# djamahl99/findnpropagate

Measured on AMD Instinct MI355X. Metric: NuScenes scenes/s (30k pts, Transfusion voxel backbone), higher is better.
Workload: dtype bf16

## Files before the change

findnpropagate_amd/csrc/rankgrid.h:

```cpp
#pragma once
#include "common.h"
#include <stdlib.h>

struct RankGridDims {
    int B, D, H, W;
    int bd, bh, bw;
    int th, tw;
};

__host__ __device__ inline RankGridDims fnp_make_dims(int B, int D, int H, int W) {
    RankGridDims g;
    g.B = B; g.D = D; g.H = H; g.W = W;
    g.bd = (D + 3) >> 2; g.bh = (H + 3) >> 2; g.bw = (W + 3) >> 2;
    g.th = (g.bh + 7) >> 3; g.tw = (g.bw + 7) >> 3;
    return g;
}

__host__ __device__ inline long long fnp_num_blocks(const RankGridDims &g) {
    return (long long)g.B * g.th * g.tw * 64 * g.bd;
}

struct RG {
    RankGridDims d;
    unsigned long long *bits;
// ... 141 lines not shown
    }
    __syncthreads();
    if (go.ctr) {
        if (tid < kCntTab && tab->cnt.key[tid] != 0u) {
            rg_count_global(go, tab->cnt.key[tid] - 1u, tab->cnt.val[tid]);
            tab->cnt.key[tid] = tab->cnt.val[tid] = 0u;
        }
        __syncthreads();
    }
}


__device__ __forceinline__ int rg_lookup(const RG &g, int b, int z, int y, int x) {
    const long long blk = rg_block_of(g.d, b, z, y, x);
    const unsigned long long w = g.bits[blk];
    const int bit = rg_bit_of(z, y, x);
    if (!((w >> bit) & 1ull)) return -1;
    const int r = (int)g.base[blk] + __popcll(w & ((1ull << bit) - 1ull));
    return g.perm ? g.perm[r] : r;
}

template <int KZ, int KY, int KX, bool DEFER = true>
__device__ __forceinline__ void nbr_row(const RG &g, int b, int loz, int loy, int lox, int *strip, int sstride, unsigned *mask_out = nullptr) {
    const int bz0 = loz >> 2, by0 = loy >> 2, bx0 = lox >> 2;
    unsigned long long w[2][2][2];
    unsigned base[2][2][2];
#pragma unroll
    for (int cy = 0; cy < 2; ++cy)
#pragma unroll
        for (int cx = 0; cx < 2; ++cx) {
            const int by = by0 + cy, bx = bx0 + cx;
            const bool need_yx = (cy == 0 || ((loy + KY - 1) >> 2) != by0) && (cx == 0 || ((lox + KX - 1) >> 2) != bx0);
            const bool in_yx = by >= 0 && by < g.d.bh && bx >= 0 && bx < g.d.bw;
            const unsigned col = (rg_morton3((unsigned)by & 7u) << 1) | rg_morton3((unsigned)bx & 7u);
            const long long colbase = ((((long long)b * g.d.th + (by >> 3)) * g.d.tw + (bx >> 3)) * 64 + col) * g.d.bd;
#pragma unroll
            for (int cz = 0; cz < 2; ++cz) {
                const int bz = bz0 + cz;
                const bool need = need_yx && (cz == 0 || ((loz + KZ - 1) >> 2) != bz0);
                const bool in = in_yx && bz >= 0 && bz < g.d.bd;
                unsigned long long ww = 0ull;
                unsigned bb = 0u;
                if (need && in) {
                    ww = g.bits[colbase + bz];
                    bb = g.base[colbase + bz];
                }
                w[cz][cy][cx] = ww;
                base[cz][cy][cx] = bb;
            }
        }
    constexpr int K = KZ * KY * KX;
    unsigned msk = 0u;
    int rk[DEFER ? K : 1];
    const int px0 = lox & 3;
    unsigned bitx[KX], mA[KX];
    bool selx[KX], vx[KX];
#pragma unroll
    for (int jx = 0; jx < KX; ++jx) {
        const int pj = px0 + jx, x = lox + jx;
        selx[jx] = pj >= 4;
        bitx[jx] = 1u << pj;
        mA[jx] = selx[jx] ? ((bitx[jx] - 1u) & 0xF0u) : (bitx[jx] - 1u);
        vx[jx] = x >= 0 && x < g.d.W;
    }
#pragma unroll
    for (int jz = 0; jz < KZ; ++jz) {
        const int z = loz + jz;
        const bool cz = (z >> 2) != bz0;
        const bool vz = z >= 0 && z < g.d.D;
        unsigned long long wz[2][2];
        unsigned bzv[2][2];
#pragma unroll
        for (int cy = 0; cy < 2; ++cy)
#pragma unroll
            for (int cx = 0; cx < 2; ++cx) {
                wz[cy][cx] = cz ? w[1][cy][cx] : w[0][cy][cx];
                bzv[cy][cx] = cz ? base[1][cy][cx] : base[0][cy][cx];
            }
#pragma unroll
        for (int jy = 0; jy < KY; ++jy) {
            const int y = loy + jy;
            const bool cy = (y >> 2) != by0;
            const bool vy = vz && y >= 0 && y < g.d.H;
            const unsigned long long wy0 = cy ? wz[1][0] : wz[0][0], wy1 = cy ? wz[1][1] : wz[0][1];
            const unsigned by0v = cy ? bzv[1][0] : bzv[0][0], by1v = cy ? bzv[1][1] : bzv[0][1];
            const int line = ((z & 3) << 4) | ((y & 3) << 2);
            const unsigned long long below = (1ull << line) - 1ull;
            const unsigned pre0 = by0v + (unsigned)__popcll(wy0 & below), pre1 = by1v + (unsigned)__popcll(wy1 & below);
            const unsigned lb = ((unsigned)(wy0 >> line) & 0xFu) | (((unsigned)(wy1 >> line) & 0xFu) << 4);
#pragma unroll
            for (int jx = 0; jx < KX; ++jx) {
                const bool hit = vy && vx[jx] && (lb & bitx[jx]) != 0u;
                const int r = (int)((selx[jx] ? pre1 : pre0) + (unsigned)__popc(lb & mA[jx]));
                const int e = (jz * KY + jy) * KX + jx;
                if constexpr (DEFER) {
                    rk[e] = hit ? r : -1;
                } else {
                    int rr = hit ? r : -1;
                    if (g.perm && hit) rr = g.perm[r];
                    strip[e * sstride] = rr;
                    if (mask_out && hit) msk |= 1u << (e & 31);
                }
            }
        }
    }
    if constexpr (DEFER) {
        if (g.perm) {
            int pr[K];
#pragma unroll
            for (int k = 0; k < K; ++k) pr[k] = g.perm[rk[k] < 0 ? 0 : rk[k]];
#pragma unroll
            for (int k = 0; k < K; ++k) rk[k] = rk[k] < 0 ? -1 : pr[k];
        }
#pragma unroll
        for (int k = 0; k < K; ++k) {
            strip[k * sstride] = rk[k];
            if (mask_out && rk[k] >= 0) msk |= 1u << (k & 31);
        }
    }
    if (mask_out) *mask_out = msk;
}


template <int K>
__device__ __forceinline__ void nbr_flush(const int *__restrict__ strip_wave, int o0, int n, int cap, int *__restrict__ nbr) {
    const int lane = fnp_lane();
    if ((cap & 3) == 0) {
#pragma unroll
        for (int j = 0; j < (K * 16 + 63) / 64; ++j) {
            const int e = j * 64 + lane, k = e >> 4, c = e & 15;
            if (k < K) {
                const int4 v = *reinterpret_cast<const int4 *>(strip_wave + k * 64 + c * 4);
                const int o = o0 + c * 4;
                if (o + 3 < n) *reinterpret_cast<int4 *>(nbr + (size_t)k * cap + o) = v;
                else {
                    if (o < n) nbr[(size_t)k * cap + o] = v.x;
                    if (o + 1 < n) nbr[(size_t)k * cap + o + 1] = v.y;
                    if (o + 2 < n) nbr[(size_t)k * cap + o + 2] = v.z;
                }
            }
        }
    } else {
#pragma unroll
        for (int k = 0; k < K; ++k)
            if (o0 + lane < n) nbr[(size_t)k * cap + o0 + lane] = strip_wave[k * 64 + lane];
    }
}


namespace fnp_scan {
constexpr int kTile = 4096;
int int32(const int *in, long long n, int *out, int *total, void *ws, hipStream_t s);
long long workspace_bytes(long long n);
int rank_grid(const RG &g, int *total, void *ws, hipStream_t s, int *out_coords = nullptr, int cap_out = 0, bool counted = false);
long long rank_grid_workspace_bytes(long long nsum);
}
```

findnpropagate_amd/csrc/scan.hip:

```cpp
#include "rankgrid.h"
#include <cstdint>
#include <type_traits>

namespace {

constexpr int kThreads = 256;
constexpr int kItems = fnp_scan::kTile / kThreads;

struct LoadInt {
    const int *p;
    __device__ __forceinline__ unsigned operator()(long long i) const { return (unsigned)p[i]; }
};

__device__ __forceinline__ unsigned wave_inclusive(unsigned v) {
    const int lane = fnp_lane();
#pragma unroll
    for (int d = 1; d < 64; d <<= 1) {
        const unsigned t = __shfl_up(v, d);
        if (lane >= d) v += t;
    }
    return v;
}

__device__ __forceinline__ unsigned block_exclusive(unsigned v, unsigned *wsum, unsigned &total) {
    const int wave = threadIdx.x >> 6, lane = fnp_lane();
    const unsigned inc = wave_inclusive(v);
    __syncthreads();
    if (lane == 63) wsum[wave] = inc;
    __syncthreads();
    unsigned off = 0;
#pragma unroll
    for (int w = 0; w < kThreads / 64; ++w) {
        const unsigned s = wsum[w];
        if (w < wave) off += s;
    }
    total = wsum[0] + wsum[1] + wsum[2] + wsum[3];
    return off + inc - v;
}

template <class L>
__global__ __launch_bounds__(kThreads) void tile_reduce_kernel(L load, long long n, unsigned *__restrict__ partial) {
    __shared__ unsigned wsum[4];
    const long long base = (long long)blockIdx.x * fnp_scan::kTile;
    unsigned s = 0;
#pragma unroll
    for (int j = 0; j < kItems; ++j) {
        const long long i = base + j * kThreads + threadIdx.x;
        if (i < n) s += load(i);
    }
    unsigned total;
    block_exclusive(s, wsum, total);
    if (threadIdx.x == 0) partial[blockIdx.x] = total;
}

__global__ __launch_bounds__(kThreads) void partial_scan_kernel(unsigned *__restrict__ partial, int np,
                                                                int *__restrict__ total_out) {
    __shared__ unsigned wsum[4];
    unsigned carry = 0;
    for (int base = 0; base < np; base += kThreads) {
        const int i = base + threadIdx.x;
        const unsigned v = i < np ? partial[i] : 0u;
        unsigned total;
        const unsigned ex = block_exclusive(v, wsum, total);
        if (i < np) partial[i] = carry + ex;
        carry += total;
    }
    if (threadIdx.x == 0) *total_out = (int)carry;
}

template <class L, class TOut>
__global__ __launch_bounds__(kThreads) void tile_scan_kernel(L load, long long n, const unsigned *__restrict__ partial,
                                                             TOut *__restrict__ out) {
    __shared__ unsigned wsum[4];
    const long long base = (long long)blockIdx.x * fnp_scan::kTile;
    unsigned carry = partial[blockIdx.x];
#pragma unroll 1
    for (int j = 0; j < kItems; ++j) {
        const long long i = base + j * kThreads + threadIdx.x;
        const unsigned v = i < n ? load(i) : 0u;
        unsigned total;
        const unsigned ex = block_exclusive(v, wsum, total);
        if (i < n) out[i] = (TOut)(carry + ex);
        carry += total;
    }
}

constexpr int kSmallTiles = 16;
__global__ __launch_bounds__(kThreads) void small_scan_kernel(const int *__restrict__ in, int n, int *__restrict__ out, int *__restrict__ total_out) {
    __shared__ unsigned wsum[4];
    const int base = blockIdx.x * fnp_scan::kTile;
    const int4 *in4 = reinterpret_cast<const int4 *>(in);
    unsigned s0 = 0, s1 = 0, s2 = 0, s3 = 0;
    for (int c = threadIdx.x; c < base / 4; c += 4 * kThreads) {
        const int4 a = in4[c];
        const int4 b = c + kThreads < base / 4 ? in4[c + kThreads] : make_int4(0, 0, 0, 0);
        const int4 d = c + 2 * kThreads < base / 4 ? in4[c + 2 * kThreads] : make_int4(0, 0, 0, 0);
        const int4 e = c + 3 * kThreads < base / 4 ? in4[c + 3 * kThreads] : make_int4(0, 0, 0, 0);
        s0 += (unsigned)(a.x + a.y + a.z + a.w);
        s1 += (unsigned)(b.x + b.y + b.z + b.w);
        s2 += (unsigned)(d.x + d.y + d.z + d.w);
        s3 += (unsigned)(e.x + e.y + e.z + e.w);
    }
    unsigned carry;
    block_exclusive(s0 + s1 + s2 + s3, wsum, carry);
    int4 v[kItems / 4];
#pragma unroll
    for (int j = 0; j < kItems / 4; ++j) {
        const int i = base + (j * kThreads + threadIdx.x) * 4;
        v[j] = make_int4(0, 0, 0, 0);
        if (i + 3 < n) v[j] = in4[i >> 2];
        else {
            if (i < n) v[j].x = in[i];
            if (i + 1 < n) v[j].y = in[i + 1];
            if (i + 2 < n) v[j].z = in[i + 2];
        }
    }
#pragma unroll
    for (int j = 0; j < kItems / 4; ++j) {
        const int i = base + (j * kThreads + threadIdx.x) * 4;
        unsigned tot;
        const unsigned ex = carry + block_exclusive((unsigned)(v[j].x + v[j].y + v[j].z + v[j].w), wsum, tot);
        const int4 o = make_int4((int)ex, (int)(ex + (unsigned)v[j].x), (int)(ex + (unsigned)(v[j].x + v[j].y)), (int)(ex + (unsigned)(v[j].x + v[j].y + v[j].z)));
        if (i + 3 < n) reinterpret_cast<int4 *>(out)[i >> 2] = o;
        else {
            if (i < n) out[i] = o.x;
            if (i + 1 < n) out[i + 1] = o.y;
            if (i + 2 < n) out[i + 2] = o.z;
        }
        carry += tot;
    }
    if (blockIdx.x == gridDim.x - 1 && threadIdx.x == 0) *total_out = (int)carry;
}

template <class L, class TOut>
int run_scan(L load, long long n, TOut *out, int *total, void *ws, hipStream_t s) {
    if (n < 0 || !total) return FNP_ERR_ARG;
    if (n == 0) {
        return fnp_fill_words(total, 1, 0u, s);
    }
    if (!out || !ws) return FNP_ERR_ARG;
    const int tiles = fnp_divup(n, fnp_scan::kTile);
    if constexpr (std::is_same<L, LoadInt>::value && std::is_same<TOut, int>::value) {
        if (tiles <= kSmallTiles && (const int *)out != load.p && (((uintptr_t)load.p | (uintptr_t)out) & 15) == 0) {
            hipLaunchKernelGGL(small_scan_kernel, dim3(tiles), dim3(kThreads), 0, s, load.p, (int)n, out, total);
            FNP_LAUNCH_CHECK();
            return FNP_OK;
        }
    }
    unsigned *partial = (unsigned *)ws;
    hipLaunchKernelGGL(HIP_KERNEL_NAME(tile_reduce_kernel<L>), dim3(tiles), dim3(kThreads), 0, s, load, n, partial);
    FNP_LAUNCH_CHECK();
    hipLaunchKernelGGL(partial_scan_kernel, dim3(1), dim3(kThreads), 0, s, partial, tiles, total);
    FNP_LAUNCH_CHECK();
    hipLaunchKernelGGL(HIP_KERNEL_NAME(tile_scan_kernel<L, TOut>), dim3(tiles), dim3(kThreads), 0, s, load, n, partial, out);
    FNP_LAUNCH_CHECK();
    return FNP_OK;
}

__device__ __forceinline__ unsigned wave_sum(unsigned v) {
#pragma unroll
    for (int d = 32; d >= 1; d >>= 1) v += __shfl_xor(v, d);
    return v;
}
__device__ __forceinline__ unsigned long long readlane64(unsigned long long v, int l) {
    const unsigned lo = __builtin_amdgcn_readlane((int)(unsigned)v, l), hi = __builtin_amdgcn_readlane((int)(unsigned)(v >> 32), l);
    return ((unsigned long long)hi << 32) | lo;
}

__global__ __launch_bounds__(kThreads) void rank_totals_kernel(const unsigned *__restrict__ cnt, long long nunits,
                                                               unsigned *__restrict__ gtot, unsigned *__restrict__ ctot) {
    __shared__ unsigned part[16];
    const int wave = threadIdx.x >> 6, lane = fnp_lane();
    const long long c = blockIdx.x;
#pragma unroll
    for (int i = 0; i < 4; ++i) {
        const long long grp = c * 16 + wave * 4 + i, U = grp * 64 + lane;
        const unsigned t = wave_sum(U < nunits ? cnt[U] : 0u);
        if (lane == 0) {
            part[wave * 4 + i] = t;
            if (grp * 64 < nunits) gtot[grp] = t;
        }
    }
    __syncthreads();
    if (threadIdx.x == 0) {
        unsigned t = 0;
#pragma unroll
        for (int i = 0; i < 16; ++i) t += part[i];
        ctot[c] = t;
    }
}

template <int PASS, int WPW>
__global__ __launch_bounds__(kThreads) void summary_pass_kernel(RG g, long long nunits, unsigned *__restrict__ cnt,
                                                                const unsigned *__restrict__ gtot,
                                                                const unsigned *__restrict__ ctot, int nchunks,
                                                                int *__restrict__ total, int cap_out,
                                                                int *__restrict__ out_coords) {
    constexpr int ROUND = WPW < 4 ? WPW : 4;
    const int lane = fnp_lane();
    const long long U = ((long long)fnp_xcd_block() * kThreads + threadIdx.x) >> 6;
    if (U >= nunits) return;
    if (PASS == 1 && U == 0) {
        unsigned t = 0;
        for (int c = lane; c < nchunks; c += 64) t += ctot[c];
        t = wave_sum(t);
        if (lane == 0) *total = (int)t;
    }
    const long long S0 = U * WPW;
    unsigned long long swl, todo;
    if (WPW == 1) {
        swl = g.summ[S0];
        todo = swl != 0ull ? 1ull : 0ull;
    } else {
        swl = (lane < WPW && S0 + lane < g.nsum) ? g.summ[S0 + lane] : 0ull;
        todo = __ballot(swl != 0ull);
    }
    if (todo == 0ull) {
        if (PASS == 0 && lane == 0) cnt[U] = 0u;
        return;
    }
    unsigned run = 0;
    if (PASS == 1) {
        const long long grp = U >> 6, chunk = U >> 10;
        unsigned p = 0;
        for (int i = lane; i < (int)chunk; i += 64) p += ctot[i];
        if (lane < (int)(grp - chunk * 16)) p += gtot[chunk * 16 + lane];
        if (lane < (int)(U - grp * 64)) p += cnt[grp * 64 + lane];
        run = wave_sum(p);
    }
    while (todo) {
        int j[ROUND];
        bool v[ROUND];
        unsigned long long bits[ROUND];
#pragma unroll
        for (int u = 0; u < ROUND; ++u) {
            v[u] = todo != 0ull;
            j[u] = v[u] ? __builtin_ctzll(todo) : 0;
            if (v[u]) todo &= todo - 1ull;
            const unsigned long long sw = WPW == 1 ? swl : readlane64(swl, j[u]);
            const bool occ = v[u] && ((sw >> lane) & 1ull);
            bits[u] = occ ? g.bits[(S0 + j[u]) * 64 + lane] : 0ull;
        }
#pragma unroll
        for (int u = 0; u < ROUND; ++u) {
            const unsigned c = (unsigned)__popcll(bits[u]);
            if (PASS == 0) {
                run += c;
            } else {
                if (!v[u]) break;
                const unsigned inc = wave_inclusive(c);
                const long long blk = (S0 + j[u]) * 64 + lane;
                int r = (int)(run + inc - c);
                if (bits[u]) {
                    g.base[blk] = (unsigned)r;
                    if (out_coords) {
                        int b, z0, y0, x0;
                        rg_decode(g.d, blk, 0, b, z0, y0, x0);
                        unsigned long long m = bits[u];
                        while (m) {
                            const int bit = __ffsll((long long)m) - 1;
                            m &= m - 1;
                            if (r < cap_out)
                                reinterpret_cast<int4 *>(out_coords)[r] = make_int4(b, z0 | (bit >> 4), y0 | ((bit >> 2) & 3), x0 | (bit & 3));
                            ++r;
                        }
                    }
                }
                if (WPW > 1) run += (unsigned)__builtin_amdgcn_readlane((int)inc, 63);
            }
        }
    }
    if (PASS == 0) {
        run = wave_sum(run);
        if (lane == 0) cnt[U] = run;
    }
}

}

namespace fnp_scan {
long long workspace_bytes(long long n) { return ((n + kTile - 1) / kTile + 1) * 4 + 64; }
int int32(const int *in, long long n, int *out, int *total, void *ws, hipStream_t s) {
    return run_scan(LoadInt{in}, n, out, total, ws, s);
}
long long rank_grid_workspace_bytes(long long nsum) {
    const long long ngroups = (nsum + 63) >> 6, nchunks = (nsum + 1023) >> 10;
    return ((nsum * 4 + 255) & ~255ll) + (((ngroups + nchunks) * 4 + 255) & ~255ll) + 256;
}
template <int WPW>
static int rank_grid_w(const RG &g, int *total, void *ws, hipStream_t s, int *out_coords, int cap_out, bool counted) {
    const long long nunits = (g.nsum + WPW - 1) / WPW;
    const long long ngroups = (nunits + 63) >> 6, nchunks = (nunits + 1023) >> 10;
    if (nchunks > 0x7fffffffll) return FNP_ERR_ARG;
    unsigned *cnt = (unsigned *)ws;
    unsigned *gtot = (unsigned *)((char *)ws + ((nunits * 4 + 255) & ~255ll));
    unsigned *ctot = gtot + ngroups;
    const int grid = fnp_divup(nunits * 64, kThreads);
    if (counted) {
        if (!g.ctr || g.wpw != WPW || g.nunits != nunits) return FNP_ERR_ARG;
        if (g.ctr_levels < 3) {
            hipLaunchKernelGGL(rank_totals_kernel, dim3((unsigned)nchunks), dim3(kThreads), 0, s, (const unsigned *)g.ctr, nunits, g.ctr + nunits,
                               g.ctr + nunits + ngroups);
            FNP_LAUNCH_CHECK();
        }
        hipLaunchKernelGGL(HIP_KERNEL_NAME(summary_pass_kernel<1, WPW>), dim3(grid), dim3(kThreads), 0, s, g, nunits, g.ctr,
                           (const unsigned *)(g.ctr + nunits), (const unsigned *)(g.ctr + nunits + ngroups), (int)nchunks, total, cap_out, out_coords);
        FNP_LAUNCH_CHECK();
        return FNP_OK;
    }
    hipLaunchKernelGGL(HIP_KERNEL_NAME(summary_pass_kernel<0, WPW>), dim3(grid), dim3(kThreads), 0, s, g, nunits, cnt,
                       (const unsigned *)nullptr, (const unsigned *)nullptr, (int)nchunks, total, 0, (int *)nullptr);
    FNP_LAUNCH_CHECK();
    hipLaunchKernelGGL(rank_totals_kernel, dim3((unsigned)nchunks), dim3(kThreads), 0, s, (const unsigned *)cnt, nunits, gtot, ctot);
    FNP_LAUNCH_CHECK();
    hipLaunchKernelGGL(HIP_KERNEL_NAME(summary_pass_kernel<1, WPW>), dim3(grid), dim3(kThreads), 0, s, g, nunits, cnt,
                       (const unsigned *)gtot, (const unsigned *)ctot, (int)nchunks, total, cap_out, out_coords);
    FNP_LAUNCH_CHECK();
    return FNP_OK;
}
int rank_grid(const RG &g, int *total, void *ws, hipStream_t s, int *out_coords, int cap_out, bool counted) {
    const int wpw = g.wpw;
    if (wpw == 64) return rank_grid_w<64>(g, total, ws, s, out_coords, cap_out, counted);
    if (wpw == 16) return rank_grid_w<16>(g, total, ws, s, out_coords, cap_out, counted);
    if (wpw == 8) return rank_grid_w<8>(g, total, ws, s, out_coords, cap_out, counted);
    return rank_grid_w<1>(g, total, ws, s, out_coords, cap_out, counted);
}
}

extern "C" int64_t fnp_rankgrid_counter_words(int B, int D, int H, int W) {
    if (B <= 0 || D <= 0 || H <= 0 || W <= 0) return 0;
    const long long nblk = fnp_num_blocks(fnp_make_dims(B, D, H, W));
    return fnp_rg_counter_words((nblk + 63) >> 6) + 64;
}

extern "C" int64_t fnp_rankgrid_workspace_bytes(int B, int D, int H, int W) {
    if (B <= 0 || D <= 0 || H <= 0 || W <= 0) return 0;
    const long long nblk = fnp_num_blocks(fnp_make_dims(B, D, H, W));
    return fnp_scan::rank_grid_workspace_bytes((nblk + 63) >> 6) + 256;
}
```

findnpropagate_amd/csrc/voxelize.hip:

```cpp
#include "rankgrid.h"

namespace {

constexpr int kThreads = 256;
constexpr int kSentinel = 0x7f7f7f7f;
constexpr int kMaxBatch = 1024;

struct VoxWs {
    long long *code;
    int *rank;
    int *flag;
    int *top;
    int *cnt;
    int *scene;
    int *n_sorted;
    int *n_first;
    int *fscan;
    void *scan_ws;
};

__host__ long long align_up(long long v) { return (v + 255) & ~255ll; }

__host__ long long carve(VoxWs &w, char *base, long long n, int B, int cap, int maxp, long long nsum) {
    long long off = 0;
    auto take = [&](long long bytes) {
        char *p = base ? base + off : nullptr;
        off += align_up(bytes);
        return p;
    };
    w.code = (long long *)take(8 * n);
    w.rank = (int *)take(4 * n);
    w.flag = (int *)take(4 * n);
    w.fscan = (int *)take(4 * n);
    w.top = (int *)take(4ll * cap * maxp);
    w.cnt = (int *)take(4ll * cap + 4);
    w.scene = (int *)take(4ll * (3 * B + 8));
    w.n_sorted = (int *)take(4);
    w.n_first = (int *)take(4);
    const long long a = fnp_scan::rank_grid_workspace_bytes(nsum), b2 = fnp_scan::workspace_bytes(n);
    w.scan_ws = take(a > b2 ? a : b2);
    return off;
}

__device__ __forceinline__ int batch_of(const int *__restrict__ off, int B, int i) {
    int lo = 0, hi = B;
    while (hi - lo > 1) {
        const int mid = (lo + hi) >> 1;
        if (off[mid] <= i) lo = mid; else hi = mid;
    }
    return lo;
}

__global__ __launch_bounds__(kThreads) void vox_mark_kernel(const float *__restrict__ pts, int n, int C,
                                                            const int *__restrict__ boff, int B, fnp_voxel_cfg cfg,
                                                            RG g, long long *__restrict__ code, int *__restrict__ cnt) {
    {
        const int z = blockIdx.x * kThreads + threadIdx.x;
        if (z <= n) cnt[z] = 0;
        if (z == 0 && (long long)gridDim.x * kThreads <= n) cnt[n] = 0;
    }
    __shared__ MarkTab tab;
    mark_tab_init(&tab, threadIdx.x, kThreads);
    const int i = blockIdx.x * kThreads + threadIdx.x;
    const int lane = fnp_lane();
    long long blk = -1;
    unsigned long long m = 0ull;
    if (i < n) {
        const float *p = pts + (size_t)i * C;
        int c[3];
        bool ok = true;
#pragma unroll
        for (int j = 0; j < 3; ++j) {
            const float q = (p[j] - cfg.range_min[j]) / cfg.voxel_size[j];
            const float f = floorf(q);
            ok = ok && (f >= 0.f) && (f < (float)cfg.grid[j]);
            c[j] = (int)f;
        }
        long long cd = -1;
        if (ok) {
            const int i0 = __builtin_amdgcn_readfirstlane(i);
            int b = batch_of(boff, B, i0);
            if (b + 1 < B && i >= boff[b + 1]) b = batch_of(boff, B, i);
            blk = rg_block_of(g.d, b, c[2], c[1], c[0]);
            const int bit = rg_bit_of(c[2], c[1], c[0]);
            m = 1ull << bit;
            cd = (blk << 6) | bit;
        }
        code[i] = cd;
    }
#pragma unroll
    for (int d = 1; d < 64; d <<= 1) {
        const long long nb = __shfl_up(blk, d);
        const unsigned long long nm = __shfl_up(m, d);
        if (lane >= d && nb == blk) m |= nm;
    }
    const long long nxt = __shfl_down(blk, 1);
    if (blk >= 0 && (lane == 63 || nxt != blk)) mark_put(&tab, g, blk, m);
    mark_tab_flush(&tab, g, threadIdx.x, kThreads);
}

__global__ __launch_bounds__(kThreads) void vox_insert_kernel(int n, int maxp, int cap,
                                                              const unsigned long long *__restrict__ bits,
                                                              const unsigned *__restrict__ base,
                                                              const long long *__restrict__ code,
                                                              int *__restrict__ rank, int *__restrict__ top, int *__restrict__ cnt,
                                                              int *__restrict__ crowded, int *__restrict__ late) {
    const int i = blockIdx.x * kThreads + threadIdx.x;
    if (i >= n) return;
    late[i] = 0;
    const long long cd = code[i];
    int r = -1;
    if (cd >= 0) {
        const long long blk = cd >> 6;
        const int bit = (int)(cd & 63);
        r = (int)base[blk] + __popcll(bits[blk] & ((1ull << bit) - 1ull));
        if (r >= cap) r = -1;
    }
    rank[i] = r;
    if (r < 0) return;
    const int s = atomicAdd(&cnt[r], 1);
    if (s < maxp) {
        top[(size_t)r * maxp + s] = i;
    } else {
        late[i] = 1;
        if (s == maxp) *crowded = 1;
    }
}

__global__ __launch_bounds__(kThreads) void vox_crowded_insert_kernel(int n, int maxp, const int *__restrict__ rank, const int *__restrict__ late,
                                                                     int *__restrict__ top, const int *__restrict__ crowded) {
    if (*crowded == 0) return;
    const int i = blockIdx.x * kThreads + threadIdx.x;
    if (i >= n || late[i] == 0) return;
    int carry = i;
    int *slots = top + (size_t)rank[i] * maxp;
    for (int j = 0; j < maxp; ++j) {
        const int old = atomicMin(&slots[j], carry);
        carry = old > carry ? old : carry;
    }
}

__global__ __launch_bounds__(kThreads) void vox_flag_kernel(int n, int maxp, const int *__restrict__ rank,
                                                            const int *__restrict__ top, const int *__restrict__ cnt, int *__restrict__ flag) {
    const int i = fnp_xcd_block() * kThreads + threadIdx.x;
    if (i >= n) return;
    const int r = rank[i];
    int f = 0;
    if (r >= 0) {
        const int np = min(cnt[r], maxp);
        int m = kSentinel;
        for (int j = 0; j < np; ++j) m = min(m, top[(size_t)r * maxp + j]);
        f = m == i ? 1 : 0;
    }
    flag[i] = f;
}

__global__ __launch_bounds__(64) void vox_scene_kernel(const int *__restrict__ boff, int B, int n, const int *__restrict__ fc,
                                                       const int *__restrict__ n_first, int max_voxels, int cap,
                                                       int *__restrict__ scene, int *__restrict__ n_voxels) {
    int *fc_start = scene;
    int *out_base = scene + (B + 1);
    const int lane = threadIdx.x;
    const int total = *n_first;
    int acc = 0;
    for (int b0 = 0; b0 < B; b0 += 64) {
        const int b = b0 + lane;
        int c = 0;
        if (b < B) {
            const int o0 = boff[b], o1 = boff[b + 1];
            const int f0 = (o0 < n) ? fc[o0] : total, f1 = (o1 < n) ? fc[o1] : total;
            fc_start[b] = f0;
            if (b == B - 1) fc_start[B] = f1;
            c = min(f1 - f0, max_voxels);
        }
        int inc = c;
#pragma unroll
        for (int d = 1; d < 64; d <<= 1) {
            const int t = __shfl_up(inc, d);
            if (lane >= d) inc += t;
        }
        if (b < B) out_base[b] = acc + inc - c;
        acc += __shfl(inc, 63);
    }
    if (lane == 0) {
        out_base[B] = acc;
        scene[2 * (B + 1)] = 0;
        *n_voxels = acc;
    }
}

struct CellPts {
    const int *slots;
    int np, s0, s1;
    __device__ __forceinline__ int next_above(int prev) const {
        if (np <= 2) {
            const int a = s0, b = np == 2 ? s1 : kSentinel;
            const int lo = a < b ? a : b, hi = a < b ? b : a;
            return lo > prev ? lo : hi;
        }
        int m = kSentinel;
        for (int j = 0; j < np; ++j) {
            const int v = slots[j];
            m = (v > prev && v < m) ? v : m;
        }
        return m;
    }
};

__device__ __forceinline__ void vox_write_row(const float *__restrict__ pts, int C, int maxp, const CellPts &cp, int p0, int r, int id,
                                              int bb, int z, int y, int x, int *__restrict__ perm, int *__restrict__ coords,
                                              int *__restrict__ num_points, float *__restrict__ mean, float *__restrict__ voxels) {
    const int np = cp.np;
    auto next_above = [&](int prev) -> int { return cp.next_above(prev); };
    perm[r] = id;
    reinterpret_cast<int4 *>(coords)[id] = make_int4(bb, z, y, x);
    num_points[id] = np;
    const float norm = (float)(np < 1 ? 1 : np);
    if ((C == 5 || C == 4) && maxp < 16) {
        typedef float f4u __attribute__((ext_vector_type(4), aligned(4)));
        f4u s4 = {0.f, 0.f, 0.f, 0.f};
        float part[4] = {0.f, 0.f, 0.f, 0.f}, tl[3] = {0.f, 0.f, 0.f};
        const int P4 = maxp & ~3;
        int pi = p0;
        for (int j = 0; j < np; ++j) {
            const float *pr = pts + (size_t)pi * C;
            const f4u v4 = *reinterpret_cast<const f4u *>(pr);
            const float v1 = C == 5 ? pr[4] : 0.f;
            if (j + 1 < np) pi = next_above(pi);
            s4 += v4;
#pragma unroll
            for (int k = 0; k < 4; ++k) part[k] += (j < P4 && (j & 3) == k) ? v1 : 0.f;
#pragma unroll
            for (int k = 0; k < 3; ++k) tl[k] = (j == P4 + k) ? v1 : tl[k];
        }
        float *mo = mean + (size_t)id * C;
        f4u m4 = {s4[0] / norm, s4[1] / norm, s4[2] / norm, s4[3] / norm};
        *reinterpret_cast<f4u *>(mo) = m4;
        if (C == 5) {
            float s1f = part[0];
#pragma unroll
            for (int k = 0; k < 3; ++k) s1f += (P4 + k < maxp) ? tl[k] : 0.f;
            s1f += part[1];
            s1f += part[2];
            s1f += part[3];
            mo[4] = s1f / norm;
        }
    } else {
        for (int c = 0; c < C; ++c) {
            const bool ilp = C < 8 && c >= (C / 4) * 4;
            const int nsum = ilp ? 4 : 1, size = ilp ? maxp / 4 : maxp;
            int lp = 0;
            while ((1 << lp) < size) ++lp;
            lp = C >= 8 ? 30 : max(4, lp / 4);
            const int mask = (1 << lp) - 1;
            float acc[4][4];
#pragma unroll
            for (int k = 0; k < 4; ++k)
#pragma unroll
                for (int l = 0; l < 4; ++l) acc[k][l] = 0.f;
            float tail = 0.f;
            bool tail_started = false;
            int pi = p0;
            for (int j = 0; j < maxp; ++j) {
                const float v = j < np ? pts[(size_t)pi * C + c] : 0.f;
                if (j + 1 < np) pi = next_above(pi);
                if (j < size * nsum) {
                    const int e = j / nsum + 1;
#pragma unroll
                    for (int k = 0; k < 4; ++k) {
                        if (k != (ilp ? (j & 3) : 0)) continue;
                        acc[k][0] += v;
                        if ((e & mask) == 0) {
#pragma unroll
                            for (int l = 1; l < 4; ++l) {
                                acc[k][l] += acc[k][l - 1];
                                acc[k][l - 1] = 0.f;
                                if ((e & (mask << (l * lp))) != 0) break;
                            }
                        }
                    }
                } else {
                    if (!tail_started) {
#pragma unroll
                        for (int l = 1; l < 4; ++l) acc[0][0] += acc[0][l];
                        tail = acc[0][0];
                        tail_started = true;
                    }
                    tail += v;
                }
            }
            float sacc;
            if (ilp) {
                if (!tail_started) {
#pragma unroll
                    for (int l = 1; l < 4; ++l) acc[0][0] += acc[0][l];
                    tail = acc[0][0];
                }
                sacc = tail;
#pragma unroll
                for (int k = 1; k < 4; ++k) {
#pragma unroll
                    for (int l = 1; l < 4; ++l) acc[k][0] += acc[k][l];
                    sacc += acc[k][0];
                }
            } else {
#pragma unroll
                for (int l = 1; l < 4; ++l) acc[0][0] += acc[0][l];
// ... 24 lines not shown
                                                                   float *__restrict__ voxels, int *__restrict__ n_cells,
                                                                   int *__restrict__ n_dropped) {
    const int ns = min(*n_sorted, cap);
    const int *fc_start = scene;
    const int *out_base = scene + (B + 1);
    if (n_cells && blockIdx.x == 0 && threadIdx.x == 0) *n_cells = ns;
    for (int r = ns + blockIdx.x * kThreads + threadIdx.x; r < cap; r += gridDim.x * kThreads) perm[r] = -1;
    const int i = (int)fnp_xcd_block() * kThreads + threadIdx.x;
    if (i >= n) return;
    const int r = rank[i];
    if (r < 0) return;
    const int f0 = fc[i], f1 = i + 1 < n ? fc[i + 1] : *n_first;
    if (f1 == f0) return;
    const long long cd = code[i];
    int bb, z, y, x;
    rg_decode(g, cd >> 6, (int)(cd & 63), bb, z, y, x);
    const int srank = f0 - fc_start[bb];
    const int id = out_base[bb] + srank;
    if (srank >= max_voxels || id >= cap) {
        perm[r] = -1;
        if (n_cells) {
            const int t = out_base[B] + atomicAdd(n_dropped, 1);
            if (t < cap) reinterpret_cast<int4 *>(coords)[t] = make_int4(bb, z, y, x);
        }
        return;
    }
    CellPts cp;
    cp.slots = top + (size_t)r * maxp;
    cp.np = min(cnt[r], maxp);
    cp.s0 = i;
    cp.s1 = kSentinel;
    if (cp.np == 2) {
        const int a = cp.slots[0], b = cp.slots[1];
        cp.s1 = a == i ? b : a;
    }
    vox_write_row(pts, C, maxp, cp, i, r, id, bb, z, y, x, perm, coords, num_points, mean, voxels);
}

__device__ __forceinline__ bool coord_ok(const RankGridDims &g, const int4 &c) {
    return c.x >= 0 && c.x < g.B && c.y >= 0 && c.y < g.D && c.z >= 0 && c.z < g.H && c.w >= 0 && c.w < g.W;
}

__device__ __forceinline__ void rg_zero_counters(const RG &g, long long first, long long stride) {
    if (!g.ctr) return;
    const long long words = g.nunits + ((g.nunits + 63) >> 6) + ((g.nunits + 1023) >> 10);
    for (long long i = first; i < words; i += stride) g.ctr[i] = 0u;
}

template <bool CLEAR>
__global__ __launch_bounds__(kThreads) void rg_mark_coords_kernel(const int *__restrict__ coords,
                                                                  const int *__restrict__ n_rows, int cap, RG g) {
    const int n = min(*n_rows, cap);
    for (int i = blockIdx.x * kThreads + threadIdx.x; i < n; i += gridDim.x * kThreads) {
        const int4 c = reinterpret_cast<const int4 *>(coords)[i];
        if (!coord_ok(g.d, c)) continue;
        const long long blk = rg_block_of(g.d, c.x, c.y, c.z, c.w);
        if (CLEAR) {
            g.bits[blk] = 0ull;
            g.summ[blk >> 6] = 0ull;
        } else {
            rg_mark(g, blk, rg_bit_of(c.y, c.z, c.w));
        }
    }
    if (CLEAR) rg_zero_counters(g, (long long)blockIdx.x * kThreads + threadIdx.x, (long long)gridDim.x * kThreads);
}

__global__ __launch_bounds__(kThreads) void rg_perm_kernel(const int *__restrict__ coords, const int *__restrict__ n_rows,
                                                           int cap, RG g) {
    const int n = min(*n_rows, cap);
    RG lookup = g;
    lookup.perm = nullptr;
    for (int i = blockIdx.x * kThreads + threadIdx.x; i < n; i += gridDim.x * kThreads) {
        const int4 c = reinterpret_cast<const int4 *>(coords)[i];
        if (!coord_ok(g.d, c)) continue;
        const int r = rg_lookup(lookup, c.x, c.y, c.z, c.w);
        if (r >= 0 && r < cap) g.perm[r] = i;
    }
}

}

extern "C" int64_t fnp_rankgrid_num_blocks(int B, int D, int H, int W) {
    if (B <= 0 || D <= 0 || H <= 0 || W <= 0) return 0;
    return fnp_num_blocks(fnp_make_dims(B, D, H, W));
}
extern "C" int64_t fnp_rankgrid_num_summary(int B, int D, int H, int W) {
    return (fnp_rankgrid_num_blocks(B, D, H, W) + 63) >> 6;
}

static bool grid_covers(const fnp_voxel_cfg *cfg, const fnp_rankgrid *g) {
    return g->D >= cfg->grid[2] && g->H >= cfg->grid[1] && g->W >= cfg->grid[0];
}

extern "C" int64_t fnp_voxelize_workspace_bytes(int64_t n_points, const fnp_voxel_cfg *cfg, const fnp_rankgrid *grid) {
    if (!cfg || n_points < 0 || !grid || grid->B <= 0 || !grid_covers(cfg, grid)) return FNP_ERR_ARG;
    VoxWs w;
    const RankGridDims g = fnp_make_dims(grid->B, grid->D, grid->H, grid->W);
    const long long n = n_points > 0 ? n_points : 1;
    return carve(w, nullptr, n, grid->B, (int)n, cfg->max_points, (fnp_num_blocks(g) + 63) >> 6);
}

__global__ __launch_bounds__(kThreads) void stage_points_kernel(const float *__restrict__ src, long long n_words, long long n_prev_words, float pad,
                                                                float *__restrict__ dst, const int *__restrict__ off_src, int n_off,
                                                                int *__restrict__ off_dst) {
    const long long i = (long long)blockIdx.x * kThreads + threadIdx.x;
    if (i < n_words) dst[i] = src[i];
    else if (i < n_prev_words) dst[i] = pad;
    if (i < n_off) off_dst[i] = off_src[i];
}
extern "C" int fnp_stage_points(const float *points, int64_t n_points, int64_t n_prev_points, int num_features, float pad, float *dst_points,
                                const int *batch_offsets, int n_offsets, int *dst_offsets, fnp_stream_t stream) {
    if (n_points < 0 || n_prev_points < 0 || num_features <= 0 || !dst_points || n_offsets < 0 || (n_points > 0 && !points) ||
        (n_offsets > 0 && (!batch_offsets || !dst_offsets)))
        return FNP_ERR_ARG;
    const long long nw = (long long)n_points * num_features, pw = (long long)n_prev_points * num_features;
    const long long span = nw > pw ? nw : pw;
    const long long items = span > n_offsets ? span : n_offsets;
    if (items == 0) return FNP_OK;
    if (items > (long long)kThreads * 0x7fffffff) return FNP_ERR_ARG;
    hipLaunchKernelGGL(stage_points_kernel, dim3((unsigned)((items + kThreads - 1) / kThreads)), dim3(kThreads), 0, (hipStream_t)stream, points, nw, pw, pad,
                       dst_points, batch_offsets, n_offsets, dst_offsets);
    FNP_LAUNCH_CHECK();
    return FNP_OK;
}

extern "C" int fnp_voxelize(const float *points, int n, const int *batch_offsets, const fnp_voxel_cfg *cfg,
                            const fnp_rankgrid *grid, void *workspace, int64_t workspace_bytes, int *coords,
                            int *num_points, float *mean_feats, float *voxels, int *n_voxels, int *n_cells, int cap,
                            fnp_stream_t stream) {
    hipStream_t s = (hipStream_t)stream;
    if (!cfg || n < 0 || cap <= 0 || !n_voxels || !fnp_rg_valid(grid, true) || grid->B > kMaxBatch || !grid_covers(cfg, grid))
        return FNP_ERR_ARG;
    if (cfg->num_features < 3 || cfg->max_points <= 0 || cfg->max_points > 64 || cfg->max_voxels <= 0) return FNP_ERR_ARG;
    if (n == 0) {
        int frc = fnp_fill_words(n_voxels, 1, 0u, s);
        if (!frc && n_cells) frc = fnp_fill_words(n_cells, 1, 0u, s);
        return frc;
    }
    if (!points || !batch_offsets || !workspace || !coords || !num_points || !mean_feats) return FNP_ERR_ARG;
    if (cap < n) return FNP_ERR_ARG;
    const RG g = fnp_rg_view(grid);
    const int B = grid->B;
    VoxWs w;
    const long long need = carve(w, (char *)workspace, n, B, n, cfg->max_points, g.nsum);
    if (need > workspace_bytes) return FNP_ERR_WORKSPACE;
    const int maxp = cfg->max_points, C = cfg->num_features;
    const int pgrid = fnp_divup(n, kThreads);

    hipLaunchKernelGGL(vox_mark_kernel, dim3(pgrid), dim3(kThreads), 0, s, points, n, C, batch_offsets, B, *cfg, g, w.code, w.cnt);
    FNP_LAUNCH_CHECK();
    int rc = fnp_scan::rank_grid(g, w.n_sorted, w.scan_ws, s, nullptr, 0, g.ctr != nullptr);
    if (rc) return rc;
    hipLaunchKernelGGL(vox_insert_kernel, dim3(pgrid), dim3(kThreads), 0, s, n, maxp, n,
                       (const unsigned long long *)g.bits, (const unsigned *)g.base, w.code, w.rank, w.top, w.cnt, w.cnt + n, w.flag);
    FNP_LAUNCH_CHECK();
    hipLaunchKernelGGL(vox_crowded_insert_kernel, dim3(pgrid), dim3(kThreads), 0, s, n, maxp, (const int *)w.rank, (const int *)w.flag, w.top, (const int *)(w.cnt + n));
    FNP_LAUNCH_CHECK();
    hipLaunchKernelGGL(vox_flag_kernel, dim3(pgrid), dim3(kThreads), 0, s, n, maxp, w.rank, w.top, (const int *)w.cnt, w.flag);
    FNP_LAUNCH_CHECK();
    rc = fnp_scan::int32(w.flag, n, w.fscan, w.n_first, w.scan_ws, s);
    if (rc) return rc;
    hipLaunchKernelGGL(vox_scene_kernel, dim3(1), dim3(64), 0, s, batch_offsets, B, n, w.fscan, w.n_first,
                       cfg->max_voxels, cap, w.scene, n_voxels);
    FNP_LAUNCH_CHECK();
    hipLaunchKernelGGL(vox_emit_points_kernel, dim3(pgrid), dim3(kThreads), 0, s, points, n, C, maxp, batch_offsets, B, cfg->max_voxels,
                       g.d, w.code, (const int *)w.rank, w.top, (const int *)w.cnt, w.fscan, (const int *)w.n_first, w.scene, w.n_sorted, n,
                       g.perm, coords, num_points, mean_feats, voxels, n_cells, w.scene + 2 * (B + 1));
    FNP_LAUNCH_CHECK();
    return FNP_OK;
}

extern "C" int fnp_rankgrid_build(const int *coords, const int *n_rows, int cap, const fnp_rankgrid *grid,
                                  void *workspace, int64_t workspace_bytes, fnp_stream_t stream) {
    hipStream_t s = (hipStream_t)stream;
    if (!coords || !n_rows || cap <= 0 || !fnp_rg_valid(grid) || !workspace) return FNP_ERR_ARG;
    const RG g = fnp_rg_view(grid);
    if (fnp_scan::rank_grid_workspace_bytes(g.nsum) + 256 > workspace_bytes) return FNP_ERR_WORKSPACE;
    int *total = (int *)workspace;
    void *scan_ws = (char *)workspace + 256;
    const int blocks = fnp_grid_for(cap, kThreads);
    hipLaunchKernelGGL(rg_mark_coords_kernel<false>, dim3(blocks), dim3(kThreads), 0, s, coords, n_rows, cap, g);
    FNP_LAUNCH_CHECK();
    int rc = fnp_scan::rank_grid(g, total, scan_ws, s);
    if (rc) return rc;
    if (g.perm) {
        {
            const int frc = fnp_fill_words(g.perm, cap, 0xffffffffu, s);
            if (frc) return frc;
        }
        hipLaunchKernelGGL(rg_perm_kernel, dim3(blocks), dim3(kThreads), 0, s, coords, n_rows, cap, g);
        FNP_LAUNCH_CHECK();
    }
    return FNP_OK;
}

extern "C" int fnp_rankgrid_clear(const int *coords, const int *n_rows, int cap, const fnp_rankgrid *grid,
                                  fnp_stream_t stream) {
    if (!coords || !n_rows || cap <= 0 || !fnp_rg_valid(grid)) return FNP_ERR_ARG;
    const RG g = fnp_rg_view(grid);
    hipLaunchKernelGGL(rg_mark_coords_kernel<true>, dim3(fnp_grid_for(cap, kThreads)), dim3(kThreads), 0,
                       (hipStream_t)stream, coords, n_rows, cap, g);
    FNP_LAUNCH_CHECK();
    return FNP_OK;
}

struct ClearJob {
    const int *coords, *n_rows;
    int cap;
    RG g;
};
struct ClearJobs { ClearJob j[8]; };

__global__ __launch_bounds__(kThreads) void rg_clear_multi_kernel(ClearJobs jobs) {
    const ClearJob &J = jobs.j[blockIdx.y];
    const int n = min(*J.n_rows, J.cap);
    for (int i = fnp_xcd_block() * kThreads + threadIdx.x; i < n; i += gridDim.x * kThreads) {
        const int4 c = reinterpret_cast<const int4 *>(J.coords)[i];
        if (!coord_ok(J.g.d, c)) continue;
        const long long blk = rg_block_of(J.g.d, c.x, c.y, c.z, c.w);
        J.g.bits[blk] = 0ull;
        J.g.summ[blk >> 6] = 0ull;
    }
    rg_zero_counters(J.g, blockIdx.x * kThreads + threadIdx.x, gridDim.x * kThreads);
}

extern "C" int fnp_rankgrid_clear_multi(int count, const int *const *coords, const int *const *n_rows, const int *caps,
                                        const fnp_rankgrid *grids, fnp_stream_t stream) {
    if (count <= 0 || count > 8 || !coords || !n_rows || !caps || !grids) return FNP_ERR_ARG;
    ClearJobs jobs{};
    int cap_max = 1;
    for (int i = 0; i < count; ++i) {
        if (!coords[i] || !n_rows[i] || caps[i] <= 0 || !fnp_rg_valid(&grids[i])) return FNP_ERR_ARG;
        jobs.j[i].coords = coords[i];
        jobs.j[i].n_rows = n_rows[i];
        jobs.j[i].cap = caps[i];
        jobs.j[i].g = fnp_rg_view(&grids[i]);
        if (caps[i] > cap_max) cap_max = caps[i];
    }
    const int gx = (fnp_grid_for(cap_max, kThreads, 512) + 7) & ~7;
    hipLaunchKernelGGL(rg_clear_multi_kernel, dim3(gx, count), dim3(kThreads), 0, (hipStream_t)stream, jobs);
    FNP_LAUNCH_CHECK();
    return FNP_OK;
}

__device__ __forceinline__ unsigned long long clr_readlane64(unsigned long long v, int l) {
    const unsigned lo = __builtin_amdgcn_readlane((int)(unsigned)v, l), hi = __builtin_amdgcn_readlane((int)(unsigned)(v >> 32), l);
    return ((unsigned long long)hi << 32) | lo;
}
__global__ __launch_bounds__(kThreads) void rg_clear_summary_kernel(ClearJobs jobs) {
    const RG &g = jobs.j[blockIdx.y].g;
    const int lane = fnp_lane();
    const long long nunits = (g.nsum + 63) >> 6, wstride = (long long)gridDim.x * (kThreads / 64);
    for (long long U = (long long)blockIdx.x * (kThreads / 64) + (threadIdx.x >> 6); U < nunits; U += wstride) {
        const long long S0 = U * 64;
        const unsigned long long sw = (S0 + lane < g.nsum) ? g.summ[S0 + lane] : 0ull;
        unsigned long long todo = __ballot(sw != 0ull);
        if (todo == 0ull) continue;
        while (todo) {
            const int j = __builtin_ctzll(todo);
            todo &= todo - 1ull;
            const unsigned long long swj = clr_readlane64(sw, j);
            if ((swj >> lane) & 1ull) g.bits[(S0 + j) * 64 + lane] = 0ull;
        }
        if (sw != 0ull) g.summ[S0 + lane] = 0ull;
    }
    rg_zero_counters(g, (long long)blockIdx.x * kThreads + threadIdx.x, (long long)gridDim.x * kThreads);
}

extern "C" int fnp_rankgrid_clear_summary(int count, const fnp_rankgrid *grids, fnp_stream_t stream) {
    if (count <= 0 || count > 8 || !grids) return FNP_ERR_ARG;
    ClearJobs jobs{};
    long long units_max = 1;
    for (int i = 0; i < count; ++i) {
        if (!fnp_rg_valid(&grids[i])) return FNP_ERR_ARG;
        jobs.j[i].g = fnp_rg_view(&grids[i]);
        const long long u = (jobs.j[i].g.nsum + 63) >> 6;
        if (u > units_max) units_max = u;
    }
    const int gx = (fnp_grid_for(units_max, kThreads / 64, 2048) + 7) & ~7;
    hipLaunchKernelGGL(rg_clear_summary_kernel, dim3(gx, count), dim3(kThreads), 0, (hipStream_t)stream, jobs);
    FNP_LAUNCH_CHECK();
    return FNP_OK;
}

#include <vector>

extern "C" int fnp_host_voxelize(const float *points, int n, const fnp_voxel_cfg *cfg, float *voxels, int *coords,
                                 int *num_points, int max_rows) {
    if (!cfg || n < 0 || max_rows < 0 || cfg->num_features < 3 || cfg->max_points <= 0 || (n > 0 && !points)) return FNP_ERR_ARG;
    if (n > 0 && max_rows > 0 && (!voxels || !coords || !num_points)) return FNP_ERR_ARG;
    const int C = cfg->num_features, P = cfg->max_points;
    const int cap_rows = cfg->max_voxels < max_rows ? cfg->max_voxels : max_rows;
    size_t tbl = 64;
    while (tbl < (size_t)(n > 0 ? n : 1) * 2) tbl <<= 1;
    std::vector<long long> keys(tbl, -1ll);
    std::vector<int> vals(tbl, 0);
    int m = 0;
    for (int i = 0; i < n; ++i) {
        const float *p = points + (size_t)i * C;
        int c[3];
        bool ok = true;
        for (int j = 0; j < 3; ++j) {
            const float q = (p[j] - cfg->range_min[j]) / cfg->voxel_size[j];
            const float f = floorf(q);
            ok = ok && (f >= 0.f) && (f < (float)cfg->grid[j]);
            c[j] = (int)f;
        }
        if (!ok) continue;
        const long long key = ((long long)c[2] * cfg->grid[1] + c[1]) * cfg->grid[0] + c[0];
        size_t h = (size_t)((unsigned long long)key * 0x9E3779B97F4A7C15ull) & (tbl - 1);
        while (keys[h] != -1ll && keys[h] != key) h = (h + 1) & (tbl - 1);
        int row;
        if (keys[h] == key) {
// ... 21 lines not shown
```

Measured before the change: 14030.

## Compact late points, fuse flag with tile sums, and self-compute small rank totals

Insert now appends overflowing points to a compact list with one wave-aggregated atomic per wave. The crowded-insert pass walks only that list with a capped grid and skips points that cannot displace a slot. When the flag scan needs more than one launch, the flag kernel also writes per-tile sums so the scan's reduce pass can be skipped. For small grids the rank pass computes prefix totals from the raw counts, dropping the separate totals kernel. These changes cut launches and full-array passes, at the cost of an extra workspace buffer and O(U) prefix loops per wave in the self-total path.

```diff
diff --git a/findnpropagate_amd/csrc/rankgrid.h b/findnpropagate_amd/csrc/rankgrid.h
--- a/findnpropagate_amd/csrc/rankgrid.h
+++ b/findnpropagate_amd/csrc/rankgrid.h
@@ -317,6 +317,9 @@
 constexpr int kTile = 4096;
 int int32(const int *in, long long n, int *out, int *total, void *ws, hipStream_t s);
 long long workspace_bytes(long long n);
+bool int32_is_one_launch(const int *in, long long n, const int *out);
+unsigned *tile_sums(void *ws);
+int int32_from_tile_sums(const int *in, long long n, int *out, int *total, void *ws, hipStream_t s);
 int rank_grid(const RG &g, int *total, void *ws, hipStream_t s, int *out_coords = nullptr, int cap_out = 0, bool counted = false);
 long long rank_grid_workspace_bytes(long long nsum);
 }
diff --git a/findnpropagate_amd/csrc/scan.hip b/findnpropagate_amd/csrc/scan.hip
--- a/findnpropagate_amd/csrc/scan.hip
+++ b/findnpropagate_amd/csrc/scan.hip
@@ -132,8 +132,12 @@
     if (blockIdx.x == gridDim.x - 1 && threadIdx.x == 0) *total_out = (int)carry;
 }
 
+bool small_scan_fits(const int *in, long long n, const int *out) {
+    return n > 0 && fnp_divup(n, fnp_scan::kTile) <= kSmallTiles && out != in && (((uintptr_t)in | (uintptr_t)out) & 15) == 0;
+}
+
 template <class L, class TOut>
-int run_scan(L load, long long n, TOut *out, int *total, void *ws, hipStream_t s) {
+int run_scan(L load, long long n, TOut *out, int *total, void *ws, hipStream_t s, bool have_sums = false) {
     if (n < 0 || !total) return FNP_ERR_ARG;
     if (n == 0) {
         return fnp_fill_words(total, 1, 0u, s);
@@ -141,15 +145,17 @@
     if (!out || !ws) return FNP_ERR_ARG;
     const int tiles = fnp_divup(n, fnp_scan::kTile);
     if constexpr (std::is_same<L, LoadInt>::value && std::is_same<TOut, int>::value) {
-        if (tiles <= kSmallTiles && (const int *)out != load.p && (((uintptr_t)load.p | (uintptr_t)out) & 15) == 0) {
+        if (!have_sums && small_scan_fits(load.p, n, (const int *)out)) {
             hipLaunchKernelGGL(small_scan_kernel, dim3(tiles), dim3(kThreads), 0, s, load.p, (int)n, out, total);
             FNP_LAUNCH_CHECK();
             return FNP_OK;
         }
     }
     unsigned *partial = (unsigned *)ws;
-    hipLaunchKernelGGL(HIP_KERNEL_NAME(tile_reduce_kernel<L>), dim3(tiles), dim3(kThreads), 0, s, load, n, partial);
-    FNP_LAUNCH_CHECK();
+    if (!have_sums) {
+        hipLaunchKernelGGL(HIP_KERNEL_NAME(tile_reduce_kernel<L>), dim3(tiles), dim3(kThreads), 0, s, load, n, partial);
+        FNP_LAUNCH_CHECK();
+    }
     hipLaunchKernelGGL(partial_scan_kernel, dim3(1), dim3(kThreads), 0, s, partial, tiles, total);
     FNP_LAUNCH_CHECK();
     hipLaunchKernelGGL(HIP_KERNEL_NAME(tile_scan_kernel<L, TOut>), dim3(tiles), dim3(kThreads), 0, s, load, n, partial, out);
@@ -200,9 +206,11 @@
     const int lane = fnp_lane();
     const long long U = ((long long)fnp_xcd_block() * kThreads + threadIdx.x) >> 6;
     if (U >= nunits) return;
+    const bool self_totals = PASS == 1 && gtot == nullptr;
     if (PASS == 1 && U == 0) {
         unsigned t = 0;
-        for (int c = lane; c < nchunks; c += 64) t += ctot[c];
+        if (self_totals) for (long long u = lane; u < nunits; u += 64) t += cnt[u];
+        else for (int c = lane; c < nchunks; c += 64) t += ctot[c];
         t = wave_sum(t);
         if (lane == 0) *total = (int)t;
     }
@@ -223,9 +231,13 @@
     if (PASS == 1) {
         const long long grp = U >> 6, chunk = U >> 10;
         unsigned p = 0;
-        for (int i = lane; i < (int)chunk; i += 64) p += ctot[i];
-        if (lane < (int)(grp - chunk * 16)) p += gtot[chunk * 16 + lane];
-        if (lane < (int)(U - grp * 64)) p += cnt[grp * 64 + lane];
+        if (self_totals) {
+            for (long long u = lane; u < U; u += 64) p += cnt[u];
+        } else {
+            for (int i = lane; i < (int)chunk; i += 64) p += ctot[i];
+            if (lane < (int)(grp - chunk * 16)) p += gtot[chunk * 16 + lane];
+            if (lane < (int)(U - grp * 64)) p += cnt[grp * 64 + lane];
+        }
         run = wave_sum(p);
     }
     while (todo) {
@@ -283,10 +295,16 @@
 int int32(const int *in, long long n, int *out, int *total, void *ws, hipStream_t s) {
     return run_scan(LoadInt{in}, n, out, total, ws, s);
 }
+bool int32_is_one_launch(const int *in, long long n, const int *out) { return small_scan_fits(in, n, out); }
+unsigned *tile_sums(void *ws) { return (unsigned *)ws; }
+int int32_from_tile_sums(const int *in, long long n, int *out, int *total, void *ws, hipStream_t s) {
+    return run_scan(LoadInt{in}, n, out, total, ws, s, true);
+}
 long long rank_grid_workspace_bytes(long long nsum) {
     const long long ngroups = (nsum + 63) >> 6, nchunks = (nsum + 1023) >> 10;
     return ((nsum * 4 + 255) & ~255ll) + (((ngroups + nchunks) * 4 + 255) & ~255ll) + 256;
 }
+constexpr long long kSelfTotalUnits = 1024;
 template <int WPW>
 static int rank_grid_w(const RG &g, int *total, void *ws, hipStream_t s, int *out_coords, int cap_out, bool counted) {
     const long long nunits = (g.nsum + WPW - 1) / WPW;
@@ -298,13 +316,15 @@
     const int grid = fnp_divup(nunits * 64, kThreads);
     if (counted) {
         if (!g.ctr || g.wpw != WPW || g.nunits != nunits) return FNP_ERR_ARG;
-        if (g.ctr_levels < 3) {
+        const bool self_totals = g.ctr_levels < 3 && nunits <= kSelfTotalUnits;
+        if (g.ctr_levels < 3 && !self_totals) {
             hipLaunchKernelGGL(rank_totals_kernel, dim3((unsigned)nchunks), dim3(kThreads), 0, s, (const unsigned *)g.ctr, nunits, g.ctr + nunits,
                                g.ctr + nunits + ngroups);
             FNP_LAUNCH_CHECK();
         }
         hipLaunchKernelGGL(HIP_KERNEL_NAME(summary_pass_kernel<1, WPW>), dim3(grid), dim3(kThreads), 0, s, g, nunits, g.ctr,
-                           (const unsigned *)(g.ctr + nunits), (const unsigned *)(g.ctr + nunits + ngroups), (int)nchunks, total, cap_out, out_coords);
+                           self_totals ? (const unsigned *)nullptr : (const unsigned *)(g.ctr + nunits), (const unsigned *)(g.ctr + nunits + ngroups),
+                           (int)nchunks, total, cap_out, out_coords);
         FNP_LAUNCH_CHECK();
         return FNP_OK;
     }
diff --git a/findnpropagate_amd/csrc/voxelize.hip b/findnpropagate_amd/csrc/voxelize.hip
--- a/findnpropagate_amd/csrc/voxelize.hip
+++ b/findnpropagate_amd/csrc/voxelize.hip
@@ -12,6 +12,7 @@
     int *flag;
     int *top;
     int *cnt;
+    int *late;
     int *scene;
     int *n_sorted;
     int *n_first;
@@ -34,6 +35,7 @@
     w.fscan = (int *)take(4 * n);
     w.top = (int *)take(4ll * cap * maxp);
     w.cnt = (int *)take(4ll * cap + 4);
+    w.late = (int *)take(4 * n);
     w.scene = (int *)take(4ll * (3 * B + 8));
     w.n_sorted = (int *)take(4);
     w.n_first = (int *)take(4);
@@ -104,55 +106,94 @@
                                                               const unsigned *__restrict__ base,
                                                               const long long *__restrict__ code,
                                                               int *__restrict__ rank, int *__restrict__ top, int *__restrict__ cnt,
-                                                              int *__restrict__ crowded, int *__restrict__ late) {
+                                                              int *__restrict__ n_late, int *__restrict__ late) {
     const int i = blockIdx.x * kThreads + threadIdx.x;
-    if (i >= n) return;
-    late[i] = 0;
-    const long long cd = code[i];
-    int r = -1;
-    if (cd >= 0) {
-        const long long blk = cd >> 6;
-        const int bit = (int)(cd & 63);
-        r = (int)base[blk] + __popcll(bits[blk] & ((1ull << bit) - 1ull));
-        if (r >= cap) r = -1;
-    }
-    rank[i] = r;
-    if (r < 0) return;
-    const int s = atomicAdd(&cnt[r], 1);
-    if (s < maxp) {
-        top[(size_t)r * maxp + s] = i;
-    } else {
-        late[i] = 1;
-        if (s == maxp) *crowded = 1;
-    }
-}
-
+    bool is_late = false;
+    if (i < n) {
+        const long long cd = code[i];
+        int r = -1;
+        if (cd >= 0) {
+            const long long blk = cd >> 6;
+            const int bit = (int)(cd & 63);
+            r = (int)base[blk] + __popcll(bits[blk] & ((1ull << bit) - 1ull));
+            if (r >= cap) r = -1;
+        }
+        rank[i] = r;
+        if (r >= 0) {
+            const int s = atomicAdd(&cnt[r], 1);
+            if (s < maxp) top[(size_t)r * maxp + s] = i;
+            else is_late = true;
+        }
+    }
+    const unsigned long long lm = __ballot(is_late);
+    if (lm == 0ull) return;
+    const int lane = fnp_lane(), leader = __builtin_ctzll(lm);
+    int at = 0;
+    if (lane == leader) at = atomicAdd(n_late, __popcll(lm));
+    at = __shfl(at, leader);
+    if (is_late) late[at + __popcll(lm & ((1ull << lane) - 1ull))] = i;
+}
+
+constexpr int kLateBlocks = 128;
 __global__ __launch_bounds__(kThreads) void vox_crowded_insert_kernel(int n, int maxp, const int *__restrict__ rank, const int *__restrict__ late,
-                                                                     int *__restrict__ top, const int *__restrict__ crowded) {
-    if (*crowded == 0) return;
-    const int i = blockIdx.x * kThreads + threadIdx.x;
-    if (i >= n || late[i] == 0) return;
-    int carry = i;
-    int *slots = top + (size_t)rank[i] * maxp;
-    for (int j = 0; j < maxp; ++j) {
-        const int old = atomicMin(&slots[j], carry);
-        carry = old > carry ? old : carry;
-    }
-}
-
+                                                                     int *__restrict__ top, const int *__restrict__ n_late) {
+    const int nl = min(*n_late, n);
+    for (int k = blockIdx.x * kThreads + threadIdx.x; k < nl; k += gridDim.x * kThreads) {
+        const int i = late[k];
+        int carry = i;
+        int *slots = top + (size_t)rank[i] * maxp;
+        int mx = -1;
+        for (int j = 0; j < maxp; ++j) mx = max(mx, slots[j]);
+        if (i > mx) continue;
+        for (int j = 0; j < maxp; ++j) {
+            const int old = atomicMin(&slots[j], carry);
+            carry = old > carry ? old : carry;
+        }
+    }
+}
+
+__device__ __forceinline__ int vox_is_first(int i, int r, int np, int maxp, const int *__restrict__ top) {
+    int m = kSentinel;
+    for (int j = 0; j < np; ++j) m = min(m, top[(size_t)r * maxp + j]);
+    return m == i ? 1 : 0;
+}
 __global__ __launch_bounds__(kThreads) void vox_flag_kernel(int n, int maxp, const int *__restrict__ rank,
                                                             const int *__restrict__ top, const int *__restrict__ cnt, int *__restrict__ flag) {
     const int i = fnp_xcd_block() * kThreads + threadIdx.x;
     if (i >= n) return;
     const int r = rank[i];
-    int f = 0;
-    if (r >= 0) {
-        const int np = min(cnt[r], maxp);
-        int m = kSentinel;
-        for (int j = 0; j < np; ++j) m = min(m, top[(size_t)r * maxp + j]);
-        f = m == i ? 1 : 0;
-    }
-    flag[i] = f;
+    flag[i] = r >= 0 ? vox_is_first(i, r, min(cnt[r], maxp), maxp, top) : 0;
+}
+constexpr int kFlagThreads = 1024, kFlagItems = fnp_scan::kTile / kFlagThreads;
+__global__ __launch_bounds__(kFlagThreads) void vox_flag_tiles_kernel(int n, int maxp, const int *__restrict__ rank,
+                                                                      const int *__restrict__ top, const int *__restrict__ cnt, int *__restrict__ flag,
+                                                                      unsigned *__restrict__ tile_sum) {
+    __shared__ unsigned wsum[kFlagThreads / 64];
+    const unsigned tile = fnp_xcd_block();
+    const long long base = (long long)tile * fnp_scan::kTile + threadIdx.x;
+    int r[kFlagItems], np[kFlagItems];
+#pragma unroll
+    for (int j = 0; j < kFlagItems; ++j) r[j] = base + j * kFlagThreads < n ? rank[base + j * kFlagThreads] : -1;
+#pragma unroll
+    for (int j = 0; j < kFlagItems; ++j) np[j] = r[j] >= 0 ? min(cnt[r[j]], maxp) : 0;
+    unsigned s = 0;
+#pragma unroll
+    for (int j = 0; j < kFlagItems; ++j) {
+        const long long i = base + j * kFlagThreads;
+        const int f = r[j] >= 0 ? vox_is_first((int)i, r[j], np[j], maxp, top) : 0;
+        if (i < n) flag[i] = f;
+        s += (unsigned)f;
+    }
+#pragma unroll
+    for (int d = 32; d >= 1; d >>= 1) s += __shfl_xor(s, d);
+    if (fnp_lane() == 0) wsum[threadIdx.x >> 6] = s;
+    __syncthreads();
+    if (threadIdx.x == 0) {
+        unsigned t = 0;
+#pragma unroll
+        for (int w = 0; w < kFlagThreads / 64; ++w) t += wsum[w];
+        tile_sum[tile] = t;
+    }
 }
 
 __global__ __launch_bounds__(64) void vox_scene_kernel(const int *__restrict__ boff, int B, int n, const int *__restrict__ fc,
@@ -483,13 +524,21 @@
     int rc = fnp_scan::rank_grid(g, w.n_sorted, w.scan_ws, s, nullptr, 0, g.ctr != nullptr);
     if (rc) return rc;
     hipLaunchKernelGGL(vox_insert_kernel, dim3(pgrid), dim3(kThreads), 0, s, n, maxp, n,
-                       (const unsigned long long *)g.bits, (const unsigned *)g.base, w.code, w.rank, w.top, w.cnt, w.cnt + n, w.flag);
-    FNP_LAUNCH_CHECK();
-    hipLaunchKernelGGL(vox_crowded_insert_kernel, dim3(pgrid), dim3(kThreads), 0, s, n, maxp, (const int *)w.rank, (const int *)w.flag, w.top, (const int *)(w.cnt + n));
-    FNP_LAUNCH_CHECK();
-    hipLaunchKernelGGL(vox_flag_kernel, dim3(pgrid), dim3(kThreads), 0, s, n, maxp, w.rank, w.top, (const int *)w.cnt, w.flag);
-    FNP_LAUNCH_CHECK();
-    rc = fnp_scan::int32(w.flag, n, w.fscan, w.n_first, w.scan_ws, s);
+                       (const unsigned long long *)g.bits, (const unsigned *)g.base, w.code, w.rank, w.top, w.cnt, w.cnt + n, w.late);
+    FNP_LAUNCH_CHECK();
+    hipLaunchKernelGGL(vox_crowded_insert_kernel, dim3(pgrid < kLateBlocks ? pgrid : kLateBlocks), dim3(kThreads), 0, s, n, maxp, (const int *)w.rank,
+                       (const int *)w.late, w.top, (const int *)(w.cnt + n));
+    FNP_LAUNCH_CHECK();
+    if (fnp_scan::int32_is_one_launch(w.flag, n, w.fscan)) {
+        hipLaunchKernelGGL(vox_flag_kernel, dim3(pgrid), dim3(kThreads), 0, s, n, maxp, w.rank, w.top, (const int *)w.cnt, w.flag);
+        FNP_LAUNCH_CHECK();
+        rc = fnp_scan::int32(w.flag, n, w.fscan, w.n_first, w.scan_ws, s);
+    } else {
+        hipLaunchKernelGGL(vox_flag_tiles_kernel, dim3(fnp_divup(n, fnp_scan::kTile)), dim3(kFlagThreads), 0, s, n, maxp, w.rank, w.top, (const int *)w.cnt,
+                           w.flag, fnp_scan::tile_sums(w.scan_ws));
+        FNP_LAUNCH_CHECK();
+        rc = fnp_scan::int32_from_tile_sums(w.flag, n, w.fscan, w.n_first, w.scan_ws, s);
+    }
     if (rc) return rc;
     hipLaunchKernelGGL(vox_scene_kernel, dim3(1), dim3(64), 0, s, batch_offsets, B, n, w.fscan, w.n_first,
                        cfg->max_voxels, cap, w.scene, n_voxels);
```

New measurement: 14060, median of 2. No clear change (+0.2%).
